# Malfoy/Brisk

Measured on AMD Instinct MI355X. Metric: distinct k-mers indexed/sec (k=63,m=21), higher is better.
Workload: dtype u64; 1 GPU; 1x MI355X: 50M synthetic 150 bp reads per GPU, k=63 m=21 b=14, uint8 counts, 15x coverage; reads_per_gpu=50000000, total_reads=50000000, part_bits=24, genome_len=500000000, parallelism=single GPU

## Files before the change

### brisk_amd/csrc/brisk_capi.hip

```cpp
#include "brisk_kernels.hip"

#include <algorithm>
#include <atomic>
#include <cerrno>
#include <chrono>
#include <cmath>
#include <cstdio>
#include <cstdlib>
#include <cstring>
#include <mutex>
#include <new>
#include <string>
#include <thread>
#include <vector>

#include <fcntl.h>
#include <sys/stat.h>
#include <unistd.h>

#include "../../include/brisk_hip.h"

#if !defined(__HIP_DEVICE_COMPILE__) && defined(__x86_64__)
#include <immintrin.h>
#define BRISK_HOST_AVX2 1
// ... 17 lines not shown
    size_t reserved = 0, mapped = 0, gran = 0;
    std::vector<hipMemGenericAllocationHandle_t> handles;
    std::vector<size_t> sizes;
};

constexpr size_t kPinBytes = 8192;
struct PendingEvent {
    int slot;
    hipEvent_t a, b;
};

struct Counters {
    struct Scan { unsigned long long n_rec; u32 overflow, pad; } scan;
    struct Touched { u32 n_touched, pad; unsigned long long need; } touched;
    struct Kmers { unsigned long long bound, n_long; } kmers;
    struct Work { u32 wc[2], n_left, n_clean; } work;
    struct Plan { u32 n_long, n_vr; } plan;
    u32 n_rerun, pad;
    unsigned long long kept;
    unsigned long long n_ovf;
    unsigned long long slice_sum;
    u32 upsert_done, pad2;
    struct Result { unsigned long long w[3]; } result;
    unsigned long long dbg_guard;
};
static_assert(sizeof(Counters::Scan) == sizeof(unsigned long long) + 2 * sizeof(u32) && sizeof(Counters::Touched) == 2 * sizeof(u32) + sizeof(unsigned long long), "ScanOut; k_touched, k_need");
static_assert(sizeof(Counters::Kmers) == 2 * sizeof(unsigned long long) && sizeof(Counters::Result) == 3 * sizeof(unsigned long long), "k_count_kmers: out[0..1]; k_checksum: out[0..2]");
static_assert(sizeof(Counters::Work) == 4 * sizeof(u32) && sizeof(Counters::Plan) == 2 * sizeof(u32), "32-bit counters throughout");
struct PinnedCounters : Counters {
    u32 n_huge;
    unsigned long long arena_used;
    unsigned long long n_rec_new;
    unsigned long long prof[3];
    unsigned long long answers;
};

}

struct brisk_hip_index {
    BriskParams P{};
    int device = 0;
    hipStream_t stream = nullptr;
    bool own_stream = false;
    std::string err;
    std::recursive_mutex call_mu;
    u64 n_parts = 0, n_buckets = 0;
    u64 max_batch_reads = 0;

    double* d_coef = nullptr;
    double* d_tabs = nullptr;
    ScanCfg scfg{};
    u64 dbg_guard_last = 0;
    bool fresh = true;
    u32 insert_waves = 4096;
    u32 scan_waves = 0;
    size_t scan_lds = 0;
    bool scan_v1 = false;
    bool entry_ids = false;
    u32 count_mode = 0;
    bool use_vmm = false;
    bool scan_hist_valid = false;
    u64 arena_limit = 0;
    VmBuf vm_keys, vm_counts, vm_ids;
    unsigned long long* d_id_counter = nullptr;
    DevBuf seq_buf;
    u64 arena_cap = 0;
// ... 407 lines not shown
    HIPCHK(h, zero_ctr(h, &h->d_ctr->touched));
    {
        ProfScope ps(h, S_TOUCHED);
        if ((rc = list_touched(h, &h->d_ctr->touched.n_touched))) return rc;
    }
    if (n_move) {
        if ((rc = ensure(h, h->parted, n_move * P.stride * 8))) return rc;
        ProfScope ps(h, S_SCATTER);
        const u64 n_slots = bl ? (u64)bl->ovf_region_cap * OVF_REGIONS : n_move;
        hipLaunchKernelGGL(k_scatter, dim3(nblocks(n_slots, 256)), dim3(256), 0, h->stream, P, bl ? (const u64*)bl->ovf : d_rec, n_move, h->d_cur32, (u64*)h->parted.p, 0,
                           (const u32*)nullptr, (u32*)nullptr, h->ix.err, bl ? bl->ovf_cnt : (const u32*)nullptr, bl ? bl->ovf_region_cap : 0u);
        if ((rc = launch_check(h, "k_scatter"))) return rc;
    }
    HIPCHK(h, fetch_ctr_sync(h, &h->d_ctr->touched.n_touched));
    const u32 n_touched = h->h_ctr->touched.n_touched;
    if (n_touched == 0) return BRISK_HIP_OK;
    static const long huge_env = getenv("BRISK_HUGE_AT") ? atol(getenv("BRISK_HUGE_AT")) : -1;
    const u32 huge_at = h->entry_ids ? 0u : huge_env >= 0 ? (u32)huge_env : 16384u;
    {
        ProfScope ps(h, S_TOUCHED);
        if ((rc = ensure(h, h->desc, (size_t)n_touched * sizeof(PartDesc)))) return rc;
        if (huge_at) {
            if ((rc = ensure(h, h->huge, (size_t)(HUGE_LIST_CAP + 1) * 4))) return rc;
            HIPCHK(h, hipMemsetAsync(h->huge.p, 0, 4, h->stream));
        }
        hipLaunchKernelGGL(k_need, dim3(std::min<u32>(nblocks(n_touched, 256), 2048)), dim3(256), 0, h->stream, h->d_hist, (bl && !n_move) ? (const u32*)nullptr : h->d_off,
                           h->d_touched, n_touched, h->ix.dir, (PartDesc*)h->desc.p, &h->d_ctr->touched.need, bl ? bl->bin_cap : 0u, huge_at, huge_at ? (u32*)h->huge.p : (u32*)nullptr,
                           (u32)HUGE_LIST_CAP);
        if (int lrc = launch_check(h, "k_need")) return lrc;
    }
// ... 16 lines not shown
        static const u32 wave_env = getenv("BRISK_INSERT_WAVES") ? (u32)atoi(getenv("BRISK_INSERT_WAVES")) : 0u;
        const bool sat = h->count_mode == BRISK_HIP_COUNTS_SATURATE;
        auto resident = [&](const void* fn, int cap_per_cu = 0) -> u32 {
            int per_cu = 0, cus = 0;
            if (hipOccupancyMaxActiveBlocksPerMultiprocessor(&per_cu, fn, 64, 0) != hipSuccess || per_cu <= 0) per_cu = 16;
            if (cap_per_cu && per_cu > cap_per_cu) per_cu = cap_per_cu;
            if (hipDeviceGetAttribute(&cus, hipDeviceAttributeMultiprocessorCount, h->device) != hipSuccess || cus <= 0) cus = 256;
            const u32 w = std::min<u32>((u32)per_cu * (u32)cus, h->insert_waves);
            static const bool dbg = getenv("BRISK_DEBUG_INSERT") != nullptr;
            if (dbg) fprintf(stderr, "[brisk_hip] k_insert: %d waves per CU x %d CUs resident, %u launched\n", per_cu, cus, wave_env ? std::min<u32>(w, wave_env) : w);
            return wave_env ? std::min<u32>(w, wave_env) : w;
        };
        static const bool generic_only = getenv("BRISK_INSERT_GENERIC") != nullptr;
        static const bool lean_off = getenv("BRISK_INSERT_LEAN") && !strcmp(getenv("BRISK_INSERT_LEAN"), "0");
        static const bool clean_off = getenv("BRISK_INSERT_CLEAN") && !strcmp(getenv("BRISK_INSERT_CLEAN"), "0");
        const bool lean = fresh && !generic_only && !lean_off && !h->entry_ids && !big && P.nw == 3 && P.kb == 49 && P.shift >= 1 && P.shift <= 4;
        if (lean) {
            if ((rc = ensure(h, h->left, (size_t)n_touched * 4))) return rc;
            static const bool dbg = getenv("BRISK_DEBUG_INSERT") != nullptr;
            if (dbg) {
                hipFuncAttributes fa{};
                int per_cu = 0;
                const void* fn = sat ? (const void*)k_insert_first<3, 49, 4, true> : (const void*)k_insert_first<3, 49, 4, false>;
                if (hipFuncGetAttributes(&fa, fn) == hipSuccess && hipOccupancyMaxActiveBlocksPerMultiprocessor(&per_cu, fn, 64, 0) == hipSuccess) {
                    fprintf(stderr, "[brisk_hip] k_insert_first: the occupancy query gives %d waves per CU, the kernel is built for at most %d\n", per_cu, 4 * WI_WAVES_PER_EU_FIRST_MAX);
                    per_cu = std::min(per_cu, 4 * WI_WAVES_PER_EU_FIRST_MAX);
                    fprintf(stderr, "[brisk_hip] k_insert_first: %d waves per CU, %d registers, %zu B of LDS, %zu B of scratch\n", per_cu, fa.numRegs, fa.sharedSizeBytes, fa.localSizeBytes);
                }
            }
        }
// ... 11 lines not shown
        else if (big) LAUNCH_INSERT_K(k_insert_big, NW, KB, SH, false)                                                                                              \
        else if (sat) LAUNCH_INSERT_K(k_insert, NW, KB, SH, true)                                                                                                   \
        else LAUNCH_INSERT_K(k_insert, NW, KB, SH, false)                                                                                                           \
    }
#define LAUNCH_INSERT_FAST(NW, KB, SH)                                                                                                                              \
    {                                                                                                                                                               \
        if (big) LAUNCH_INSERT(NW, KB, SH)                                                                                                                          \
        else if (sat) LAUNCH_INSERT_K(k_insert_fast, NW, KB, SH, true)                                                                                              \
        else LAUNCH_INSERT_K(k_insert_fast, NW, KB, SH, false)                                                                                                      \
    }
#define LAUNCH_INSERT_LEAN_K(SH, SAT)                                                                                                                               \
    {                                                                                                                                                               \
        u32* const wc = h->d_ctr->work.wc;                                                                                                                          \
        u32* const n_left = &h->d_ctr->work.n_left;                                                                                                                 \
        u32* const n_clean = clean_off ? nullptr : &h->d_ctr->work.n_clean;                                                                                         \
        body = "k_insert_first<3,49," #SH;                                                                                                                          \
        const dim3 grid(std::min<u32>(batches, resident((const void*)k_insert_first<3, 49, SH, SAT>, 4 * WI_WAVES_PER_EU_FIRST_MAX)));                                                            \
        hipLaunchKernelGGL((k_insert_first<3, 49, SH, SAT>), grid, dim3(64), 0, h->stream, P, src, (const PartDesc*)h->desc.p, n_touched, h->ix, wc,                \
                           (u32*)h->left.p, n_left, n_clean);                                                                                                       \
        if ((rc = launch_check(h, "k_insert_first"))) return rc;                                                                                                    \
        const dim3 grid2(std::min<u32>(batches, resident((const void*)k_insert_fast_listed<3, 49, SH, SAT>)));                                                     \
        hipLaunchKernelGGL((k_insert_fast_listed<3, 49, SH, SAT>), grid2, dim3(64), 0, h->stream, P, src, (const PartDesc*)h->desc.p, n_touched, h->ix, wc + 1,     \
                           (const u32*)h->left.p, (const u32*)n_left);                                                                                              \
    }
#define LAUNCH_INSERT_LEAN(SH)                                                                                                                                      \
    {                                                                                                                                                               \
        if (sat) LAUNCH_INSERT_LEAN_K(SH, true)                                                                                                                     \
        else LAUNCH_INSERT_LEAN_K(SH, false)                                                                                                                        \
    }
        if (lean && P.shift == 4) LAUNCH_INSERT_LEAN(4)
        else if (lean && P.shift == 3) LAUNCH_INSERT_LEAN(3)
        else if (lean && P.shift == 2) LAUNCH_INSERT_LEAN(2)
        else if (lean) LAUNCH_INSERT_LEAN(1)
        else if (!generic_only && P.nw == 3 && P.kb == 49 && P.shift == 4) LAUNCH_INSERT_FAST(3, 49, 4)
// ... 10 lines not shown
#undef LAUNCH_INSERT_FAST
#undef LAUNCH_INSERT
#undef LAUNCH_INSERT_K
        if ((rc = launch_check(h, big ? "k_insert_big" : "k_insert"))) return rc;
        if (h->trace) {
            std::string path = big ? "k_insert_big (in-place collapse for partitions of > 128 records)" : "k_insert", tail;
            if (lean) {
                HIPCHK(h, fetch_ctr_sync(h, &h->d_ctr->work));
                const u32 n_left = h->h_ctr->work.n_left;
                path = "k_insert_first (fresh index): " + std::to_string(n_touched - n_huge - n_left) + " partitions lean, " + std::to_string(n_left) + " left over to k_insert";
                tail = " (" + std::to_string(h->h_ctr->work.n_clean) + " table-free)";
            }
            fprintf(stderr, "[brisk_hip] path: insert of %llu records (%s layout, histogram %s) into %u partitions: %s, %u partitions to k_insert_huge%s\n", (unsigned long long)n_rec,
                    bl ? "binned" : "classic", have_hist ? "from the scan" : "counted here", n_touched, path.c_str(), n_huge, tail.c_str());
            fprintf(stderr, "[brisk_hip] body: %s,%s>%s\n", body, sat ? "sat" : "wrap", lean ? ", then k_insert_fast_listed" : "");
        }
        if (n_huge) {
            if (sat) hipLaunchKernelGGL(k_insert_huge<true>, dim3(std::min<u32>(n_huge, 256u)), dim3(HG_THREADS), 0, h->stream, P, src, (const PartDesc*)h->desc.p,
                                        (const u32*)h->huge.p + 1, (const u32*)h->huge.p, h->ix);
            else hipLaunchKernelGGL(k_insert_huge<false>, dim3(std::min<u32>(n_huge, 256u)), dim3(HG_THREADS), 0, h->stream, P, src, (const PartDesc*)h->desc.p,
                                    (const u32*)h->huge.p + 1, (const u32*)h->huge.p, h->ix);
            if ((rc = launch_check(h, "k_insert_huge"))) return rc;
        }
    }
    h->nb_skmers += n_rec;
    h->dir_snapshot_valid = false;
    return BRISK_HIP_OK;
}

int launch_scan(brisk_hip_index* h, const u32* d_packed, const u64* d_starts, u64 n_items, const ScanOut& out, bool query_mode, bool plain,
// ... 2889 lines not shown
#undef LAUNCH_DEBUG_KEYS
    if ((rc = launch_check(h, "k_debug_keys"))) return rc;
    HIPCHK(h, hipMemcpyAsync(keys, d_k, n * 8, hipMemcpyDeviceToHost, h->stream));
    HIPCHK(h, fetch_ctr_sync(h, &h->d_ctr->dbg_guard));
    h->dbg_guard_last = h->h_ctr->dbg_guard;
    return BRISK_HIP_OK;
}

BRISK_API int brisk_hip_debug_guard_count(brisk_hip_index* h, uint64_t* n_guard) {
    if (!h || !n_guard) return BRISK_HIP_EINVAL;
    std::lock_guard<std::recursive_mutex> call_lock(h->call_mu);
    *n_guard = h->dbg_guard_last;
    return BRISK_HIP_OK;
}

BRISK_API int brisk_hip_debug_host_pack(const char* bases, uint64_t n_bases, uint32_t* packed, int scalar) {
    if (n_bases && (!bases || !packed)) return BRISK_HIP_EINVAL;
    if (scalar) host_pack_scalar(bases, n_bases, packed);
    else host_pack(bases, n_bases, packed);
    return BRISK_HIP_OK;
}
#ifdef BRISK_PHASE_PROF
BRISK_API int brisk_hip_debug_scan_counts(uint64_t out[8], int reset) {
    if (hipMemcpyFromSymbol(out, HIP_SYMBOL(g_scan_cnt), 8 * 8) != hipSuccess) return BRISK_HIP_EHIP;
    if (reset) {
        uint64_t z[8] = {};
        if (hipMemcpyToSymbol(HIP_SYMBOL(g_scan_cnt), z, 8 * 8) != hipSuccess) return BRISK_HIP_EHIP;
    }
    return BRISK_HIP_OK;
}
// ... 41 lines not shown
```

### brisk_amd/csrc/brisk_insert.hip

```cpp
#ifndef ARENA_CHUNK
#define ARENA_CHUNK 16384u
#endif
#ifndef INSERT_SLOTS
#define INSERT_SLOTS 8192u
#endif
#ifndef WI_WAVES_PER_EU
#define WI_WAVES_PER_EU 4
#endif
#ifdef BRISK_PHASE_PROF
__device__ unsigned long long g_phase[16];
#define PHASE_DECL unsigned long long ph_acc[12] = {0, 0, 0, 0, 0, 0, 0, 0, 0, 0, 0, 0}; unsigned long long ph_last = __builtin_amdgcn_s_memtime(); u32 dbg_cnt[16] = {0, 0, 0, 0, 0, 0, 0, 0, 0, 0, 0, 0, 0, 0, 0, 0};
#define PHASE(i) { const unsigned long long t_ = __builtin_amdgcn_s_memtime(); ph_acc[i] += t_ - ph_last; ph_last = t_; }
__device__ unsigned long long g_cnt[16];
#define PHASE_FLUSH { PHASE(10) if (threadIdx.x == 0) { _Pragma("unroll") for (int q_ = 0; q_ < 12; q_++) atomicAdd(&g_phase[q_], ph_acc[q_]); \
                                                         _Pragma("unroll") for (int q_ = 0; q_ < 16; q_++) atomicAdd(&g_cnt[q_], (unsigned long long)dbg_cnt[q_]); } }
#define CNT(i, v) dbg_cnt[i] += (v);
#else
#define PHASE_DECL
#define PHASE(i)
#define PHASE_FLUSH
#define CNT(i, v)
#endif
struct IndexDev {
    u64* keys;
// ... 453 lines not shown
}

#ifndef FOLD_GROUPED
#define FOLD_GROUPED 1
#endif
#ifdef INSERT_ATTR_ONEROUND
#define FOLD_GROUPED_TRIPS 1u
#else
#define FOLD_GROUPED_TRIPS WI_FOLD_TRIPS
#endif
__device__ __forceinline__ u32 fold_slot(u32 ck) { return (ck * 0x9E3779B1u) >> 26; }
__device__ __forceinline__ u32 lane_fetch(u32 v, u32 a4) { return (u32)__builtin_amdgcn_ds_bpermute((int)a4, (int)v); }
__device__ __forceinline__ u64 lane_fetch64(u64 v, u32 a4) { return ((u64)lane_fetch((u32)(v >> 32), a4) << 32) | lane_fetch((u32)v, a4); }
template <u32 NW>
__device__ __forceinline__ bool fold_records_grouped(const FoldFrame& f, u32 nrec, u32 lane, u32* s_slot, u32* lead, u32* off, bool* folded_out, u32* trips, u32 ck, bool unsure,
                                                     bool* clean) {
    static_assert(WI_FOLD_TRIPS < (1u << 18), "[round | n | 63 - lane] in 32 bits: n < 256, so sv < 1 << 14");
    if (__any(unsure)) return false;
    u32 sv = lane < nrec ? f.s : 0;
    bool folded = false;
    u32 dirty = 0, heads = 0;
    *lead = lane;
    *off = 0;
    u32* my_slot = s_slot + fold_slot(ck);
    s_slot[lane] = 0;
    wave_sync();
    for (u32 t = 1; t <= FOLD_GROUPED_TRIPS; t++) {
        if (!__any(sv != 0) || heads > WI_FOLD_TRIPS) break;
        *trips += 1;
        const u32 mine = (t << 14) | sv;
        if (sv != 0) atomicMax(my_slot, mine);
// ... 11 lines not shown
        in = in && same;
        if (in) {
            sv = 0;
            if (lane != a) {
                folded = true;
                *lead = a;
                *off = i0 - i0a;
            }
        }
        const u32 meets = ((i0 - ea) & (i0a - e)) >> 31;
        dirty |= (ck_a == ck && sv != 0) ? meets : 0u;
    }
#ifndef INSERT_ATTR_ONEROUND
    if (heads > WI_FOLD_TRIPS || __any(sv != 0)) return false;
#endif
    *clean = !__any(dirty != 0);
    *folded_out = folded;
    return true;
}

template <u32 MAXI, u32 NW, u32 KB, u32 SHIFT, bool SAT, bool LISTED = false>
__device__ __forceinline__ void insert_body(const BriskParams& PP, const RecSrc& src, const PartDesc* __restrict__ desc, u32 n_touched_all, const IndexDev& ix,
                                            u32* __restrict__ work_counter, const u32* __restrict__ list = nullptr, const u32* __restrict__ n_list = nullptr) {
    const u32 n_touched = LISTED ? min(*n_list, n_touched_all) : n_touched_all;
    u64* const rec = src.rec;
    BriskParams P = PP;
    if (NW) {
        P.nw = NW;
        P.stride = NW + 1;
        P.kb = KB;
        P.shift = SHIFT;
// ... 427 lines not shown
#ifndef WI_WAVES_PER_EU_FIRST_MAX
#define WI_WAVES_PER_EU_FIRST_MAX 6
#endif
template <u32 NIL, u32 NW>
struct LeanLds {
    static constexpr u32 MAXI = 64 * NIL, TABLE = 512;
    static_assert((TABLE & (TABLE - 1)) == 0 && TABLE >= 2 * MAXI && TABLE <= 4 * MAXI, "probe table: a power of two, at most half full");
    static constexpr u32 REC_BYTES = (WI_MAX_REC * RecGeom<NW>::RS + 4) * 4;
    static constexpr u32 OFF_REC = 16 * MAXI;
    static constexpr u32 REGION = REC_BYTES > 4 * TABLE ? REC_BYTES : 4 * TABLE;
    static constexpr u32 OFF_IREC = OFF_REC + REGION, OFF_IMULT = OFF_IREC + MAXI, BYTES = OFF_IMULT + MAXI;
};
__device__ __forceinline__ unsigned long long first_lane64(unsigned long long v) {
    return ((unsigned long long)(u32)__builtin_amdgcn_readfirstlane((int)(v >> 32)) << 32) | (u32)__builtin_amdgcn_readfirstlane((int)v);
}
template <u32 NIL, u32 NW, u32 KB, u32 SHIFT, bool SAT>
__device__ __forceinline__ void insert_first_body(const BriskParams& P, const RecSrc& src, const PartDesc* __restrict__ desc, u32 n_touched, const IndexDev& ix,
                                                  u32* __restrict__ work_counter, u32* __restrict__ left_list, u32* __restrict__ n_left, u32* __restrict__ n_clean) {
    using L = LeanLds<NIL, NW>;
    constexpr u32 MAXI = L::MAXI, TABLE = L::TABLE, RS = RecGeom<NW>::RS, INFO = RecGeom<NW>::INFO, KBITS = 2 * KB + 6;
    constexpr u32 KW = KBITS + SHIFT <= 64 ? 1u : 2u;
    constexpr u32 CORE_K = 63, CORE_M = 21, CORE_B = 14, CW = CORE_K - CORE_M;
    static_assert(KB == CORE_K - CORE_B, "fold_core: the core of k63 m21 b14");
    static_assert(NIL == 2 || NIL == 3, "instance slots per lane");
    static_assert(NW >= 3 && SHIFT < 5, "the folding k63 geometries: at most 16 buckets per partition");
    static_assert(L::BYTES <= 13 * 512, "LDS per wave: 24 waves must fit a CU's 160 KiB");
    static_assert(4 * MAXI <= 16 * MAXI, "the multiplicity steps lie over the keys");
    static_assert(MAXI + (MAXI >> 2) + 8 <= ARENA_CHUNK / 8, "grow_cap(MAXI) is a small request: the host's arena reserve covers the tail a refill strands");
    __shared__ __attribute__((aligned(16))) unsigned char s_mem[L::BYTES];
    u64* s_key = (u64*)s_mem;
    u32* s_idiff = (u32*)s_mem;
    u32* s_rw = (u32*)(s_mem + L::OFF_REC);
    u32* s_tab = (u32*)(s_mem + L::OFF_REC);
    uint8_t* s_irec = s_mem + L::OFF_IREC;
    uint8_t* s_imult = s_mem + L::OFF_IMULT;

    const u32 lane = threadIdx.x;
    PHASE_DECL
    unsigned long long acur = first_lane64(ix.slot_cur[blockIdx.x]), aend = first_lane64(ix.slot_end[blockIdx.x]), garbage = 0;
    const u32 frame_end = P.suff_reduc + P.w + 1;
    const u32 core_from = (n_clean != nullptr && P.w == CW) ? P.suff_reduc : 0x100u;

    for (;;) {
        u32 t0 = 0;
        if (lane == 0) t0 = atomicAdd(work_counter, WI_BATCH);
        t0 = (u32)__builtin_amdgcn_readfirstlane((int)t0);
        if (t0 >= n_touched) break;
        const u32 t_end = min(t0 + WI_BATCH, n_touched);
        unsigned long long left_mask = 0;
        unsigned long long clean_mask = 0;
        PartDesc d = desc[t0];
        RecRegs rr = load_part_recs(P, src, d.part, d.r_begin, d.r_begin, min(d.n_rec, (u32)WI_MAX_REC), lane);

        for (u32 t = t0; t < t_end; t++) {
            const u32 tn = t + 1;
            PartDesc dn{};
            if (tn < t_end) dn = desc[tn];
            asm volatile("" ::"v"(rr.w0), "v"(rr.w1), "v"(rr.w2), "v"(rr.w3), "v"(rr.w4));
            do {
                if (ix.huge_at && d.n_inst > ix.huge_at) break;
                CNT(0, 1)
                if (d.n_exist | d.cap | (u32)(d.n_rec > WI_MAX_REC)) {
                    left_mask |= 1ull << (t - t0);
                    break;
                }
                PHASE(0)
                const u32 part = d.part, nrec = d.n_rec;
                const u64 my_hdr = NW == 3 ? rr.w3 : rr.w4;
                const u32 raw_n = lane < nrec ? hdr_n(my_hdr) : 0;
                const u32 my_mult = (my_hdr & HDR_HAS_MULT) ? (u32)(my_hdr >> 48) & 0xffu : 1u;
                const u32 info_hi = (raw_n << 10) | (hdr_idx0(my_hdr) << 18) | ((hdr_bucket(my_hdr) & ((1u << SHIFT) - 1)) << 26);
                const FoldFrame ff = fold_frame<NW, KB>(rr, my_hdr, raw_n, lane < nrec, frame_end, lane);
                wave_sync();
                if (lane < nrec) store_rec_words<NW>(s_rw + lane * RS, rr, 0);
                u32 lead = lane, lead_off = 0, dbg_trips = 0;
                const bool unsure = lane < nrec && (ff.s == 0 || hdr_idx0(my_hdr) < core_from);
                bool clean = false;
                const u32 ck = ((hdr_bucket(my_hdr) & ((1u << SHIFT) - 1)) << (2 * (KB - CW))) | fold_core<KB, CW>(ff.u);
                bool dup = false;
                if (!FOLD_GROUPED || !fold_records_grouped<NW>(ff, nrec, lane, (u32*)s_mem, &lead, &lead_off, &dup, &dbg_trips, ck, unsure, &clean))
                    dup = fold_records<NW, true>(ff, nrec, lane, &lead, &lead_off, &dbg_trips, ck, unsure, &clean);
#ifdef INSERT_ATTR_NOTABLE
                clean = true;
#endif
                const u32 my_n = (lane < nrec && !dup) ? raw_n : 0;
                const u32 x = wave_incl_scan(my_n, lane);
                const u32 ninst = (u32)__builtin_amdgcn_readlane((int)x, 63);
                if (ninst > MAXI) {
                    left_mask |= 1ull << (t - t0);
                    break;
                }
                PHASE(1)
                CNT(1, 1)
                const u32 m_first = (u32)__shfl(x - my_n, lead, 64) + lead_off;
                u32 tsize = 128;
                while (tsize < 4 * ninst && tsize < TABLE) tsize <<= 1;
                {
                    if (NIL == 2) ((uint16_t*)s_irec)[lane] = 0;
                    else {
#pragma unroll
                        for (u32 q = 0; q < NIL; q++) s_irec[q * 64 + lane] = 0;
                    }
// ... 40 lines not shown
                        }
                    }
                    if (lane < nrec) s_rw[lane * RS + INFO] = (x - my_n) | info_hi;
                }
                wave_sync();
                PHASE(2)
                CNT(3, (ninst + 63) / 64)
                CNT(4, ninst)
                CNT(5, nrec)
                CNT(11, dbg_trips)
                u32 dbg_r = 0;
                LaneInst<NIL> li;
                li.won = 0;
                u32 n_new = 0, new_rank[NIL], new_word[NIL];
                if (clean) {
                    clean_mask |= 1ull << (t - t0);
                    u32 ln = lane;
                    asm volatile("" : "+v"(ln));
                    if (ninst <= 64) expand_words_distinct<1, NW, KB, SHIFT, NIL>(ln, ninst, s_rw, s_irec, li);
                    else if (NIL == 2 || ninst <= 128) expand_words_distinct<2, NW, KB, SHIFT, NIL>(ln, ninst, s_rw, s_irec, li);
                    else expand_words_distinct<NIL, NW, KB, SHIFT, NIL>(ln, ninst, s_rw, s_irec, li);
                    n_new = ninst;
#pragma unroll
                    for (u32 it = 0; it < NIL; it++) {
                        const u32 i = it * 64 + ln;
                        new_rank[it] = i;
                        new_word[it] = (u32)s_imult[i < ninst ? i : 0] << WI_CNT_SHIFT;
                    }
                    PHASE(3)
                } else {
                    if (ninst <= 64) expand_and_dedupe_words<1, NW, KB, SHIFT, NIL, true, SAT>(lane, ninst, tsize, s_rw, s_irec, s_imult, nullptr, s_key, s_tab, &dbg_r, li);
// ... 9 lines not shown
                        if (it * 64 < ninst) {
                            const bool made = (li.won >> it) & 1;
                            if (made) new_word[it] = s_tab[li.hh[it]];
                            const unsigned long long bal = __ballot(made);
                            new_rank[it] = n_new + (u32)__popcll(bal & lanes_below(lane));
                            n_new += (u32)__popcll(bal);
                        }
                    }
                }
                wave_sync();
#ifndef INSERT_NO_EARLY_WAIT
                __builtin_amdgcn_s_waitcnt(0x0F70);
#endif
                PHASE(6)
                CNT(7, n_new)
                unsigned long long off = d.off;
                u32 cap = 0;
                if (n_new) {
                    const unsigned long long want = grow_cap(n_new);
                    if (acur + want > aend) {
                        garbage += aend - acur;
                        unsigned long long got = 0;
                        if (lane == 0) got = atomicAdd(ix.cursor, (unsigned long long)ARENA_CHUNK);
                        acur = first_lane64(got);
                        aend = acur + ARENA_CHUNK;
                    }
                    if (acur + want > ix.arena_cap) {
                        if (lane == 0) atomicOr(ix.err, 2u);
                        n_new = 0;
                    } else {
                        off = acur;
                        acur += want;
                        cap = (u32)want;
                    }
                }
                PHASE(7)
                u32 bm0 = 0;
#pragma unroll
                for (u32 it = 0; it < NIL; it++) {
                    if (it * 64 < ninst && ((li.won >> it) & 1) && n_new) {
                        const unsigned long long at = off + new_rank[it];
                        store_key<KW>(ix, at, li.klo[it], li.khi[it]);
                        ix.counts[at] = (uint8_t)count8<SAT>(new_word[it] >> WI_CNT_SHIFT);
                        const u32 bl = SHIFT ? ((u32)shr128(mk128(li.klo[it], li.khi[it]), KBITS).lo & ((1u << SHIFT) - 1)) : 0;
                        bm0 |= 1u << bl;
                    }
                }
                PHASE(8)
                bm0 = wave_or_all(bm0);
                if (lane == 0) {
                    ix.dir[part] = DirEnt{off, n_new, cap};
                    const u64 first = ((u64)part << SHIFT) >> P.ext_bits;
                    const u32 bits = bm0 << (first & 31);
                    if (bits && (!ix.bits_check || (ix.bucket_bits[first >> 5] & bits) != bits)) atomicOr(&ix.bucket_bits[first >> 5], bits);
                }
            } while (0);
            d = dn;
            if (tn < t_end) rr = load_part_recs(P, src, d.part, d.r_begin, d.r_begin, min(d.n_rec, (u32)WI_MAX_REC), lane);
            PHASE(9)
        }
        if (left_mask) {
            const u32 n = (u32)__popcll(left_mask);
            u32 at = 0;
            if (lane == 0) at = atomicAdd(n_left, n);
            at = (u32)__builtin_amdgcn_readfirstlane((int)at);
            u32 ln = lane;
            asm volatile("" : "+v"(ln));
            if ((left_mask >> ln) & 1) left_list[at + (u32)__popcll(left_mask & lanes_below(ln))] = t0 + ln;
        }
        if (clean_mask && n_clean && lane == 0) atomicAdd(n_clean, (u32)__popcll(clean_mask));
    }
    PHASE_FLUSH
    if (lane == 0) {
        ix.slot_cur[blockIdx.x] = acur;
        ix.slot_end[blockIdx.x] = aend;
        if (garbage) atomicAdd(&ix.stats[3], garbage);
    }
}
template <u32 NW, u32 KB, u32 SHIFT, bool SAT = false, u32 NIL = NI_LEAN>
__global__ void __launch_bounds__(64) __attribute__((amdgpu_waves_per_eu(WI_WAVES_PER_EU_FIRST, WI_WAVES_PER_EU_FIRST_MAX))) k_insert_first(BriskParams P, RecSrc src, const PartDesc* __restrict__ desc,
                                                                                                          u32 n_touched, IndexDev ix, u32* __restrict__ work_counter,
                                                                                                          u32* __restrict__ left_list, u32* __restrict__ n_left, u32* __restrict__ n_clean) {
    insert_first_body<NIL, NW, KB, SHIFT, SAT>(P, src, desc, n_touched, ix, work_counter, left_list, n_left, n_clean);
}

__global__ void __launch_bounds__(256) k_bucket_bits(BriskParams P, IndexDev ix, u32 n_parts) {
    const u32 kbits = 2 * P.kb + 6;
    for (u32 part = blockIdx.x; part < n_parts; part += gridDim.x) {
        const u32 cnt = ix.dir[part].cnt;
        const unsigned long long off = ix.dir[part].off;
        for (u32 e = threadIdx.x; e < cnt; e += blockDim.x) {
            const u128x key = load_key(ix, off + e);
            const u32 bucket = (part << P.shift) | ((u32)shr128(key, kbits).lo & ((1u << P.shift) - 1));
            const u32 bit = 1u << (bucket & 31);
            if (!(ix.bucket_bits[bucket >> 5] & bit)) atomicOr(&ix.bucket_bits[bucket >> 5], bit);
        }
    }
}
// ... 229 lines not shown
```

### brisk_amd/hipapi.py

```python
from __future__ import annotations

import atexit
import ctypes as C
import math
import os
import subprocess
import sys
import weakref
from typing import Optional, Sequence, Tuple

import numpy as np

HERE = os.path.dirname(os.path.abspath(__file__))
ROOT = os.path.dirname(HERE)
_LIB_NAME = os.environ.get("BRISK_HIP_LIB", "libbrisk_hip.so")

STATUS = {0: "OK", 1: "EINVAL", 2: "EUNSUPPORTED", 3: "EHIP", 4: "ENOMEM", 5: "ECAPACITY", 6: "ENODEVICE", 7: "EIO", 8: "EFORMAT"}
ECAPACITY = 5


class BriskHipError(RuntimeError):
    def __init__(self, code: int, msg: str = ""):
        self.code = code
        super().__init__(f"brisk_hip: {STATUS.get(code, code)} {msg}".strip())
# ... 72 lines not shown

class _JointWindow(C.Structure):
    _fields_ = [(n, C.c_uint32) for n in ("min_self", "max_self", "min_other", "max_other", "keep_absent", "reserved")]


JOINT_ABSENT = 256
JOINT_STATES = 257

_u64p = np.ctypeslib.ndpointer(dtype=np.uint64, flags="C_CONTIGUOUS")
_u8p = np.ctypeslib.ndpointer(dtype=np.uint8, flags="C_CONTIGUOUS")

SYMBOLS = [
    "brisk_hip_abi_version", "brisk_hip_create", "brisk_hip_destroy", "brisk_hip_clear", "brisk_hip_last_error", "brisk_hip_sync",
    "brisk_hip_get_layout", "brisk_hip_insert_reads", "brisk_hip_insert_packed", "brisk_hip_get_reads", "brisk_hip_lookup",
    "brisk_hip_enumerate", "brisk_hip_stats", "brisk_hip_memory_info", "brisk_hip_insert_slack", "brisk_hip_reallocate", "brisk_hip_checksum", "brisk_hip_scan_packed", "brisk_hip_scan_bound", "brisk_hip_route_records",
    "brisk_hip_get_packed", "brisk_hip_get_kmers", "brisk_hip_get_kmers_packed", "brisk_hip_insert_records", "brisk_hip_set_owner_cuts", "brisk_hip_export_hist", "brisk_hip_export_hist_add", "brisk_hip_insert_records_hist", "brisk_hip_scan_query", "brisk_hip_route_tagged", "brisk_hip_query_records", "brisk_hip_pack_ascii", "brisk_hip_synth_reads", "brisk_hip_debug_order_keys", "brisk_hip_debug_guard_count", "brisk_hip_scan_sequence", "brisk_hip_upsert_kmers", "brisk_hip_find_kmers",
    "brisk_hip_enumerate_ids", "brisk_hip_count_spectrum", "brisk_hip_enumerate_range", "brisk_hip_prune",
    "brisk_hip_read_profile_reads", "brisk_hip_read_profile_packed",
    "brisk_hip_scan_kmers", "brisk_hip_record_kmers", "brisk_hip_answer_records", "brisk_hip_place_answers", "brisk_hip_profile_slots",
    "brisk_hip_select_intervals", "brisk_hip_extract_packed", "brisk_hip_trim_packed", "brisk_hip_trim_reads", "brisk_hip_unpack_ascii",
    "brisk_hip_intake_ascii", "brisk_hip_intake_reads", "brisk_hip_insert_raw_reads",
    "brisk_hip_fragment_intervals", "brisk_hip_pair_intervals", "brisk_hip_compose_intervals", "brisk_hip_extract_pairs_packed",
    "brisk_hip_trim_pairs_packed", "brisk_hip_trim_pairs_reads", "brisk_hip_clean_pairs_ascii", "brisk_hip_clean_pairs_reads",
    "brisk_hip_merge", "brisk_hip_intersect", "brisk_hip_subtract", "brisk_hip_compare", "brisk_hip_joint_spectrum", "brisk_hip_filter_joint", "brisk_hip_snapshot_info_read", "brisk_hip_save", "brisk_hip_load",
    "brisk_hip_profile_enable",
    "brisk_hip_profile_read", "brisk_hip_profile_reset",
]

_lib = None


# ... 923 lines not shown
        dts = (np.uint64, np.uint64, np.uint8, np.uint32)
        return tuple(np.concatenate(a) if a else np.zeros(0, dt) for a, dt in zip(out, dts))

    def debug_order_keys(self, mmers, exact: bool = False) -> np.ndarray:
        x = np.ascontiguousarray(mmers, np.uint64)
        out = np.zeros(max(len(x), 1), np.uint64)
        self._chk(self.L.brisk_hip_debug_order_keys(self.h, x, len(x), 1 if exact else 0, out))
        return out[: len(x)]

    def debug_guard_count(self) -> int:
        n = C.c_uint64(0)
        self.L.brisk_hip_debug_guard_count.argtypes = [C.c_void_p, C.POINTER(C.c_uint64)]
        self._chk(self.L.brisk_hip_debug_guard_count(self.h, C.byref(n)))
        return int(n.value)

    def profile_enable(self, on: bool = True):
        self._chk(self.L.brisk_hip_profile_enable(self.h, 1 if on else 0))

    def profile_reset(self):
        self._chk(self.L.brisk_hip_profile_reset(self.h))

    def profile_read(self) -> dict:
        n = C.c_uint32()
        names = (C.c_char_p * 16)()
        launches = (C.c_uint64 * 16)()
        ms = (C.c_double * 16)()
        self._chk(self.L.brisk_hip_profile_read(self.h, C.byref(n), names, launches, ms))
        return {names[i].decode(): {"launches": launches[i], "ms": ms[i]} for i in range(n.value)}
```

### include/brisk_hip.h

```cpp
#ifndef BRISK_HIP_H
#define BRISK_HIP_H

#include <stddef.h>
#include <stdint.h>

#ifdef __cplusplus
extern "C" {
#endif

#define BRISK_HIP_ABI_VERSION 4

enum {
    BRISK_HIP_OK = 0,
    BRISK_HIP_EINVAL = 1,
    BRISK_HIP_EUNSUPPORTED = 2,
    BRISK_HIP_EHIP = 3,
    BRISK_HIP_ENOMEM = 4,
    BRISK_HIP_ECAPACITY = 5,
    BRISK_HIP_ENODEVICE = 6,
    BRISK_HIP_EIO = 7,
    BRISK_HIP_EFORMAT = 8
};

typedef struct brisk_hip_index brisk_hip_index;
// ... 251 lines not shown
int brisk_hip_upsert_kmers(brisk_hip_index *h, const uint64_t *kmer_lo, const uint64_t *kmer_hi, const uint8_t *minimizer_idx,
                           uint64_t n, uint32_t *ids, uint8_t *newly);
int brisk_hip_find_kmers(brisk_hip_index *h, const uint64_t *kmer_lo, const uint64_t *kmer_hi, const uint8_t *minimizer_idx,
                         uint64_t n, uint32_t *ids);
int brisk_hip_enumerate_ids(brisk_hip_index *h, uint64_t *cursor, uint64_t *out_lo, uint64_t *out_hi,
                            uint8_t *out_minimizer_idx, uint32_t *out_ids, uint64_t cap, uint64_t *n_out);

int brisk_hip_pack_ascii(brisk_hip_index *h, const char *d_bases, uint64_t n_bases, uint32_t *d_packed);
int brisk_hip_unpack_ascii(brisk_hip_index *h, const uint32_t *d_packed, uint64_t first_nt, uint64_t n_nts, char *d_bases);
int brisk_hip_synth_reads(brisk_hip_index *h, uint64_t genome_len, uint64_t first_read, uint64_t n_reads,
                          uint32_t read_len, uint64_t seed_g, uint64_t seed_r,
                          uint32_t *d_packed, uint64_t *d_starts);

int brisk_hip_debug_order_keys(brisk_hip_index *h, const uint64_t *mmers, uint64_t n, int exact, uint64_t *keys);
int brisk_hip_debug_guard_count(brisk_hip_index *h, uint64_t *n_guard);

#define BRISK_HIP_PROFILE_SLOTS 16
int brisk_hip_profile_enable(brisk_hip_index *h, int on);
int brisk_hip_profile_read(brisk_hip_index *h, uint32_t *n_slots, const char **names, uint64_t *launches, double *ms);
int brisk_hip_profile_reset(brisk_hip_index *h);

#ifdef __cplusplus
}
#endif
#endif
```

Before: 33.91 billion k-mers/s.

## Pair adjacent small fresh partitions into one wave pass in k_insert_first

In the lean first-insert kernel, two consecutive fresh partitions whose combined record count fits in one wave are now loaded and folded together, with a partition bit added to the fold key so their records stay apart. If both fold cleanly and fit the instance limit, both partitions are processed and written in a single iteration, and the loop advances by two. Otherwise the code falls back to the first partition alone. The aim is to reduce idle lanes and per-partition overhead when many partitions hold only a few records, at the cost of extra branching, register pressure and refold work when a pair fails. Debug accessors for touched partitions and directory entries are also added.

```diff
diff --git a/brisk_amd/csrc/brisk_capi.hip b/brisk_amd/csrc/brisk_capi.hip
--- a/brisk_amd/csrc/brisk_capi.hip
+++ b/brisk_amd/csrc/brisk_capi.hip
@@ -55,7 +55,7 @@
     struct Scan { unsigned long long n_rec; u32 overflow, pad; } scan;
     struct Touched { u32 n_touched, pad; unsigned long long need; } touched;
     struct Kmers { unsigned long long bound, n_long; } kmers;
-    struct Work { u32 wc[2], n_left, n_clean; } work;
+    struct Work { u32 wc[2], n_left, n_clean, n_pair, pad; } work;
     struct Plan { u32 n_long, n_vr; } plan;
     u32 n_rerun, pad;
     unsigned long long kept;
@@ -67,7 +67,7 @@
 };
 static_assert(sizeof(Counters::Scan) == sizeof(unsigned long long) + 2 * sizeof(u32) && sizeof(Counters::Touched) == 2 * sizeof(u32) + sizeof(unsigned long long), "ScanOut; k_touched, k_need");
 static_assert(sizeof(Counters::Kmers) == 2 * sizeof(unsigned long long) && sizeof(Counters::Result) == 3 * sizeof(unsigned long long), "k_count_kmers: out[0..1]; k_checksum: out[0..2]");
-static_assert(sizeof(Counters::Work) == 4 * sizeof(u32) && sizeof(Counters::Plan) == 2 * sizeof(u32), "32-bit counters throughout");
+static_assert(sizeof(Counters::Work) == 6 * sizeof(u32) && sizeof(Counters::Plan) == 2 * sizeof(u32), "32-bit counters throughout");
 struct PinnedCounters : Counters {
     u32 n_huge;
     unsigned long long arena_used;
@@ -91,6 +91,7 @@
     double* d_coef = nullptr;
     double* d_tabs = nullptr;
     ScanCfg scfg{};
+    u32 dbg_touched_last = 0;
     u64 dbg_guard_last = 0;
     bool fresh = true;
     u32 insert_waves = 4096;
@@ -528,6 +529,7 @@
     }
     HIPCHK(h, fetch_ctr_sync(h, &h->d_ctr->touched.n_touched));
     const u32 n_touched = h->h_ctr->touched.n_touched;
+    h->dbg_touched_last = n_touched;
     if (n_touched == 0) return BRISK_HIP_OK;
     static const long huge_env = getenv("BRISK_HUGE_AT") ? atol(getenv("BRISK_HUGE_AT")) : -1;
     const u32 huge_at = h->entry_ids ? 0u : huge_env >= 0 ? (u32)huge_env : 16384u;
@@ -574,6 +576,7 @@
         static const bool generic_only = getenv("BRISK_INSERT_GENERIC") != nullptr;
         static const bool lean_off = getenv("BRISK_INSERT_LEAN") && !strcmp(getenv("BRISK_INSERT_LEAN"), "0");
         static const bool clean_off = getenv("BRISK_INSERT_CLEAN") && !strcmp(getenv("BRISK_INSERT_CLEAN"), "0");
+        static const bool pair_off = getenv("BRISK_INSERT_PAIR") && !strcmp(getenv("BRISK_INSERT_PAIR"), "0");
         const bool lean = fresh && !generic_only && !lean_off && !h->entry_ids && !big && P.nw == 3 && P.kb == 49 && P.shift >= 1 && P.shift <= 4;
         if (lean) {
             if ((rc = ensure(h, h->left, (size_t)n_touched * 4))) return rc;
@@ -615,10 +618,11 @@
         u32* const wc = h->d_ctr->work.wc;                                                                                                                          \
         u32* const n_left = &h->d_ctr->work.n_left;                                                                                                                 \
         u32* const n_clean = clean_off ? nullptr : &h->d_ctr->work.n_clean;                                                                                         \
+        u32* const n_pair = (clean_off || pair_off) ? nullptr : &h->d_ctr->work.n_pair;                                                                             \
         body = "k_insert_first<3,49," #SH;                                                                                                                          \
         const dim3 grid(std::min<u32>(batches, resident((const void*)k_insert_first<3, 49, SH, SAT>, 4 * WI_WAVES_PER_EU_FIRST_MAX)));                                                            \
         hipLaunchKernelGGL((k_insert_first<3, 49, SH, SAT>), grid, dim3(64), 0, h->stream, P, src, (const PartDesc*)h->desc.p, n_touched, h->ix, wc,                \
-                           (u32*)h->left.p, n_left, n_clean);                                                                                                       \
+                           (u32*)h->left.p, n_left, n_clean, n_pair);                                                                                               \
         if ((rc = launch_check(h, "k_insert_first"))) return rc;                                                                                                    \
         const dim3 grid2(std::min<u32>(batches, resident((const void*)k_insert_fast_listed<3, 49, SH, SAT>)));                                                     \
         hipLaunchKernelGGL((k_insert_fast_listed<3, 49, SH, SAT>), grid2, dim3(64), 0, h->stream, P, src, (const PartDesc*)h->desc.p, n_touched, h->ix, wc + 1,     \
@@ -659,6 +663,14 @@
             fprintf(stderr, "[brisk_hip] path: insert of %llu records (%s layout, histogram %s) into %u partitions: %s, %u partitions to k_insert_huge%s\n", (unsigned long long)n_rec,
                     bl ? "binned" : "classic", have_hist ? "from the scan" : "counted here", n_touched, path.c_str(), n_huge, tail.c_str());
             fprintf(stderr, "[brisk_hip] body: %s,%s>%s\n", body, sat ? "sat" : "wrap", lean ? ", then k_insert_fast_listed" : "");
+        }
+        if (lean) {
+            static const bool dbg = getenv("BRISK_DEBUG_INSERT") != nullptr;
+            if (dbg) {
+                HIPCHK(h, fetch_ctr_sync(h, &h->d_ctr->work));
+                fprintf(stderr, "[brisk_hip] k_insert_first: %u of %u partitions taken in pairs, %u table-free, %u left over\n", h->h_ctr->work.n_pair, n_touched,
+                        h->h_ctr->work.n_clean, h->h_ctr->work.n_left);
+            }
         }
         if (n_huge) {
             if (sat) hipLaunchKernelGGL(k_insert_huge<true>, dim3(std::min<u32>(n_huge, 256u)), dim3(HG_THREADS), 0, h->stream, P, src, (const PartDesc*)h->desc.p,
@@ -3578,6 +3590,33 @@
     return BRISK_HIP_OK;
 }
 
+BRISK_API int brisk_hip_debug_touched(brisk_hip_index* h, uint32_t* parts, uint64_t cap, uint64_t* n) {
+    if (!h || !n || (cap && !parts)) return BRISK_HIP_EINVAL;
+    HIPCHK(h, hipSetDevice(h->device));
+    std::lock_guard<std::recursive_mutex> call_lock(h->call_mu);
+    *n = h->dbg_touched_last;
+    const u64 take = std::min<u64>(cap, h->dbg_touched_last);
+    if (take) HIPCHK(h, hipMemcpyAsync(parts, h->d_touched, take * 4, hipMemcpyDeviceToHost, h->stream));
+    HIPCHK(h, hipStreamSynchronize(h->stream));
+    return BRISK_HIP_OK;
+}
+
+BRISK_API int brisk_hip_debug_directory(brisk_hip_index* h, const uint32_t* parts, uint64_t n, uint32_t* cnt, uint32_t* cap) {
+    if (!h || (n && (!parts || !cnt || !cap))) return BRISK_HIP_EINVAL;
+    HIPCHK(h, hipSetDevice(h->device));
+    std::lock_guard<std::recursive_mutex> call_lock(h->call_mu);
+    for (u64 i = 0; i < n; i++)
+        if (parts[i] >= h->n_parts) return BRISK_HIP_EINVAL;
+    std::vector<DirEnt> dir(h->n_parts);
+    HIPCHK(h, hipMemcpyAsync(dir.data(), h->ix.dir, h->n_parts * sizeof(DirEnt), hipMemcpyDeviceToHost, h->stream));
+    HIPCHK(h, hipStreamSynchronize(h->stream));
+    for (u64 i = 0; i < n; i++) {
+        cnt[i] = dir[parts[i]].cnt;
+        cap[i] = dir[parts[i]].cap;
+    }
+    return BRISK_HIP_OK;
+}
+
 BRISK_API int brisk_hip_debug_host_pack(const char* bases, uint64_t n_bases, uint32_t* packed, int scalar) {
     if (n_bases && (!bases || !packed)) return BRISK_HIP_EINVAL;
     if (scalar) host_pack_scalar(bases, n_bases, packed);
diff --git a/brisk_amd/csrc/brisk_insert.hip b/brisk_amd/csrc/brisk_insert.hip
--- a/brisk_amd/csrc/brisk_insert.hip
+++ b/brisk_amd/csrc/brisk_insert.hip
@@ -491,7 +491,7 @@
 __device__ __forceinline__ u64 lane_fetch64(u64 v, u32 a4) { return ((u64)lane_fetch((u32)(v >> 32), a4) << 32) | lane_fetch((u32)v, a4); }
 template <u32 NW>
 __device__ __forceinline__ bool fold_records_grouped(const FoldFrame& f, u32 nrec, u32 lane, u32* s_slot, u32* lead, u32* off, bool* folded_out, u32* trips, u32 ck, bool unsure,
-                                                     bool* clean) {
+                                                     bool* clean, unsigned long long* dirty_lanes = nullptr) {
     static_assert(WI_FOLD_TRIPS < (1u << 18), "[round | n | 63 - lane] in 32 bits: n < 256, so sv < 1 << 14");
     if (__any(unsure)) return false;
     u32 sv = lane < nrec ? f.s : 0;
@@ -533,7 +533,9 @@
 #ifndef INSERT_ATTR_ONEROUND
     if (heads > WI_FOLD_TRIPS || __any(sv != 0)) return false;
 #endif
-    *clean = !__any(dirty != 0);
+    const unsigned long long dl = __ballot(dirty != 0);
+    if (dirty_lanes) *dirty_lanes = dl;
+    *clean = dl == 0;
     *folded_out = folded;
     return true;
 }
@@ -991,9 +993,33 @@
 __device__ __forceinline__ unsigned long long first_lane64(unsigned long long v) {
     return ((unsigned long long)(u32)__builtin_amdgcn_readfirstlane((int)(v >> 32)) << 32) | (u32)__builtin_amdgcn_readfirstlane((int)v);
 }
+#ifndef INSERT_PAIR
+#define INSERT_PAIR 1
+#endif
+#define PAIR_B_BIT 18u
+__device__ __forceinline__ RecRegs load_pair_recs(const BriskParams& P, const RecSrc& src, u32 part_a, u32 begin_a, u32 nA, u32 part_b, u32 begin_b, u32 nB, u32 lane) {
+    RecRegs r{0, 0, 0, 0, 0};
+    const u32 in_bin = src.bin_cap ? src.bin_cap : ~0u;
+    const u64 bytes = (u64)P.stride * 8, rec0 = (u64)(uintptr_t)src.rec, ovf0 = (u64)(uintptr_t)src.ovf;
+    const u64 bin_a = rec0 + (src.bin_cap ? (u64)part_a * src.bin_cap : (u64)begin_a) * bytes, ovf_a = ovf0 + ((u64)begin_a - src.bin_cap) * bytes;
+    const u64 bin_b = rec0 + (src.bin_cap ? (u64)part_b * src.bin_cap : (u64)begin_b) * bytes, ovf_b = ovf0 + ((u64)begin_b - src.bin_cap) * bytes;
+    if (lane < nA + nB) {
+        const bool is_b = lane >= nA;
+        const u32 i = is_b ? lane - nA : lane;
+        const u64 base = i < in_bin ? (is_b ? bin_b : bin_a) : (is_b ? ovf_b : ovf_a);
+        const u64* c = (const u64*)(uintptr_t)(base + i * bytes);
+        r.w0 = c[0];
+        r.w1 = c[1];
+        if (P.stride > 2) r.w2 = c[2];
+        if (P.stride > 3) r.w3 = c[3];
+        if (P.stride > 4) r.w4 = c[4];
+    }
+    return r;
+}
 template <u32 NIL, u32 NW, u32 KB, u32 SHIFT, bool SAT>
 __device__ __forceinline__ void insert_first_body(const BriskParams& P, const RecSrc& src, const PartDesc* __restrict__ desc, u32 n_touched, const IndexDev& ix,
-                                                  u32* __restrict__ work_counter, u32* __restrict__ left_list, u32* __restrict__ n_left, u32* __restrict__ n_clean) {
+                                                  u32* __restrict__ work_counter, u32* __restrict__ left_list, u32* __restrict__ n_left, u32* __restrict__ n_clean,
+                                                  u32* __restrict__ n_pair) {
     using L = LeanLds<NIL, NW>;
     constexpr u32 MAXI = L::MAXI, TABLE = L::TABLE, RS = RecGeom<NW>::RS, INFO = RecGeom<NW>::INFO, KBITS = 2 * KB + 6;
     constexpr u32 KW = KBITS + SHIFT <= 64 ? 1u : 2u;
@@ -1017,6 +1043,20 @@
     unsigned long long acur = first_lane64(ix.slot_cur[blockIdx.x]), aend = first_lane64(ix.slot_end[blockIdx.x]), garbage = 0;
     const u32 frame_end = P.suff_reduc + P.w + 1;
     const u32 core_from = (n_clean != nullptr && P.w == CW) ? P.suff_reduc : 0x100u;
+    const bool pair_on = INSERT_PAIR && n_pair != nullptr && core_from != 0x100u;
+    auto request = [&](const PartDesc& a, u32 ta, u32 t_end, RecRegs& rr) -> u32 {
+        u32 nB = 0, part_b = 0, begin_b = 0;
+        if (pair_on && ta + 1 < t_end && !(a.n_exist | a.cap) && a.n_rec - 1u < (u32)WI_MAX_REC - 1u && !(ix.huge_at && a.n_inst > ix.huge_at)) {
+            const PartDesc b = desc[ta + 1];
+            if (!(b.n_exist | b.cap) && b.n_rec != 0 && a.n_rec + b.n_rec <= (u32)WI_MAX_REC && !(ix.huge_at && b.n_inst > ix.huge_at)) {
+                nB = b.n_rec;
+                part_b = b.part;
+                begin_b = b.r_begin;
+            }
+        }
+        rr = load_pair_recs(P, src, a.part, a.r_begin, min(a.n_rec, (u32)WI_MAX_REC), part_b, begin_b, nB, lane);
+        return nB;
+    };
 
     for (;;) {
         u32 t0 = 0;
@@ -1026,11 +1066,15 @@
         const u32 t_end = min(t0 + WI_BATCH, n_touched);
         unsigned long long left_mask = 0;
         unsigned long long clean_mask = 0;
+        u32 pairs = 0;
         PartDesc d = desc[t0];
-        RecRegs rr = load_part_recs(P, src, d.part, d.r_begin, d.r_begin, min(d.n_rec, (u32)WI_MAX_REC), lane);
-
-        for (u32 t = t0; t < t_end; t++) {
-            const u32 tn = t + 1;
+        RecRegs rr;
+        u32 nB = INSERT_PAIR ? request(d, t0, t_end, rr) : 0u;
+        if (!INSERT_PAIR) rr = load_part_recs(P, src, d.part, d.r_begin, d.r_begin, min(d.n_rec, (u32)WI_MAX_REC), lane);
+
+        for (u32 t = t0, step = 1; t < t_end; t += step) {
+            u32 tn = t + 1;
+            step = 1;
             PartDesc dn{};
             if (tn < t_end) dn = desc[tn];
             asm volatile("" ::"v"(rr.w0), "v"(rr.w1), "v"(rr.w2), "v"(rr.w3), "v"(rr.w4));
@@ -1042,7 +1086,8 @@
                     break;
                 }
                 PHASE(0)
-                const u32 part = d.part, nrec = d.n_rec;
+                const u32 part = d.part, nA = d.n_rec;
+                u32 nrec = nA + nB;
                 const u64 my_hdr = NW == 3 ? rr.w3 : rr.w4;
                 const u32 raw_n = lane < nrec ? hdr_n(my_hdr) : 0;
                 const u32 my_mult = (my_hdr & HDR_HAS_MULT) ? (u32)(my_hdr >> 48) & 0xffu : 1u;
@@ -1051,18 +1096,45 @@
                 wave_sync();
                 if (lane < nrec) store_rec_words<NW>(s_rw + lane * RS, rr, 0);
                 u32 lead = lane, lead_off = 0, dbg_trips = 0;
-                const bool unsure = lane < nrec && (ff.s == 0 || hdr_idx0(my_hdr) < core_from);
+                const bool unsure_any = ff.s == 0 || hdr_idx0(my_hdr) < core_from;
                 bool clean = false;
-                const u32 ck = ((hdr_bucket(my_hdr) & ((1u << SHIFT) - 1)) << (2 * (KB - CW))) | fold_core<KB, CW>(ff.u);
+                const u32 ck = ((hdr_bucket(my_hdr) & ((1u << SHIFT) - 1)) << (2 * (KB - CW))) | fold_core<KB, CW>(ff.u) |
+                               (INSERT_PAIR && lane >= nA ? 1u << PAIR_B_BIT : 0u);
+                static_assert(SHIFT + 2 * (KB - CW) <= PAIR_B_BIT, "ck: the partition bit lies above the routing id's low bits and the core");
                 bool dup = false;
-                if (!FOLD_GROUPED || !fold_records_grouped<NW>(ff, nrec, lane, (u32*)s_mem, &lead, &lead_off, &dup, &dbg_trips, ck, unsure, &clean))
+                unsigned long long dirty_lanes = 0;
+                for (;;) {
+                    const bool unsure = lane < nrec && unsure_any;
+                    if (FOLD_GROUPED && fold_records_grouped<NW>(ff, nrec, lane, (u32*)s_mem, &lead, &lead_off, &dup, &dbg_trips, ck, unsure, &clean, &dirty_lanes)) break;
+                    if (INSERT_PAIR && nB) {
+                        nB = 0;
+                        nrec = nA;
+                        continue;
+                    }
                     dup = fold_records<NW, true>(ff, nrec, lane, &lead, &lead_off, &dbg_trips, ck, unsure, &clean);
+                    break;
+                }
 #ifdef INSERT_ATTR_NOTABLE
                 clean = true;
 #endif
-                const u32 my_n = (lane < nrec && !dup) ? raw_n : 0;
+                u32 my_n = (lane < nrec && !dup) ? raw_n : 0;
                 const u32 x = wave_incl_scan(my_n, lane);
-                const u32 ninst = (u32)__builtin_amdgcn_readlane((int)x, 63);
+                u32 ninst = (u32)__builtin_amdgcn_readlane((int)x, 63);
+                u32 ninstA = ninst;
+                if (INSERT_PAIR && nB) {
+                    ninstA = (u32)__builtin_amdgcn_readlane((int)x, (int)(nA - 1));
+                    const bool clean_a = (dirty_lanes & ((1ull << nA) - 1)) == 0;
+                    if (clean && ninst <= MAXI) {
+                        step = 2;
+                        pairs += 2;
+                    } else {
+                        nB = 0;
+                        nrec = nA;
+                        clean = clean_a;
+                        if (lane >= nA) my_n = 0;
+                        ninst = ninstA;
+                    }
+                }
                 if (ninst > MAXI) {
                     left_mask |= 1ull << (t - t0);
                     break;
@@ -1133,7 +1205,7 @@
                 li.won = 0;
                 u32 n_new = 0, new_rank[NIL], new_word[NIL];
                 if (clean) {
-                    clean_mask |= 1ull << (t - t0);
+                    clean_mask |= (INSERT_PAIR && nB ? 3ull : 1ull) << (t - t0);
                     u32 ln = lane;
                     asm volatile("" : "+v"(ln));
                     if (ninst <= 64) expand_words_distinct<1, NW, KB, SHIFT, NIL>(ln, ninst, s_rw, s_irec, li);
@@ -1173,26 +1245,61 @@
 #endif
                 PHASE(6)
                 CNT(7, n_new)
+                auto take_slice = [&](u32& n, unsigned long long& off, u32& cap) {
+                    cap = 0;
+                    if (n) {
+                        const unsigned long long want = grow_cap(n);
+                        if (acur + want > aend) {
+                            garbage += aend - acur;
+                            unsigned long long got = 0;
+                            if (lane == 0) got = atomicAdd(ix.cursor, (unsigned long long)ARENA_CHUNK);
+                            acur = first_lane64(got);
+                            aend = acur + ARENA_CHUNK;
+                        }
+                        if (acur + want > ix.arena_cap) {
+                            if (lane == 0) atomicOr(ix.err, 2u);
+                            n = 0;
+                        } else {
+                            off = acur;
+                            acur += want;
+                            cap = (u32)want;
+                        }
+                    }
+                };
+                if (INSERT_PAIR && nB) {
+                    unsigned long long off = d.off, off_b = dn.off;
+                    u32 cap = 0, cap_b = 0, n_new_b = n_new - ninstA;
+                    n_new = ninstA;
+                    take_slice(n_new, off, cap);
+                    take_slice(n_new_b, off_b, cap_b);
+                    u32 ln = lane, bm0 = 0;
+                    asm volatile("" : "+v"(ln));
+#pragma unroll
+                    for (u32 it = 0; it < NIL; it++) {
+                        const u32 i = it * 64 + ln;
+                        const bool in_b = i >= ninstA;
+                        if (i < ninst && (in_b ? n_new_b : n_new)) {
+                            const unsigned long long at = (in_b ? off_b - ninstA : off) + i;
+                            store_key<KW>(ix, at, li.klo[it], li.khi[it]);
+                            ix.counts[at] = (uint8_t)count8<SAT>(new_word[it] >> WI_CNT_SHIFT);
+                            const u32 bl = (u32)shr128(mk128(li.klo[it], li.khi[it]), KBITS).lo & ((1u << SHIFT) - 1);
+                            bm0 |= 1u << (bl + (in_b ? 16u : 0u));
+                        }
+                    }
+                    bm0 = wave_or_all(bm0);
+                    if (ln == 0) {
+                        ix.dir[part] = DirEnt{off, n_new, cap};
+                        ix.dir[dn.part] = DirEnt{off_b, n_new_b, cap_b};
+                        const u64 first = ((u64)part << SHIFT) >> P.ext_bits, first_b = ((u64)dn.part << SHIFT) >> P.ext_bits;
+                        const u32 bits = (bm0 & 0xffffu) << (first & 31), bits_b = (bm0 >> 16) << (first_b & 31);
+                        if (bits && (!ix.bits_check || (ix.bucket_bits[first >> 5] & bits) != bits)) atomicOr(&ix.bucket_bits[first >> 5], bits);
+                        if (bits_b && (!ix.bits_check || (ix.bucket_bits[first_b >> 5] & bits_b) != bits_b)) atomicOr(&ix.bucket_bits[first_b >> 5], bits_b);
+                    }
+                    break;
+                }
                 unsigned long long off = d.off;
                 u32 cap = 0;
-                if (n_new) {
-                    const unsigned long long want = grow_cap(n_new);
-                    if (acur + want > aend) {
-                        garbage += aend - acur;
-                        unsigned long long got = 0;
-                        if (lane == 0) got = atomicAdd(ix.cursor, (unsigned long long)ARENA_CHUNK);
-                        acur = first_lane64(got);
-                        aend = acur + ARENA_CHUNK;
-                    }
-                    if (acur + want > ix.arena_cap) {
-                        if (lane == 0) atomicOr(ix.err, 2u);
-                        n_new = 0;
-                    } else {
-                        off = acur;
-                        acur += want;
-                        cap = (u32)want;
-                    }
-                }
+                take_slice(n_new, off, cap);
                 PHASE(7)
                 u32 bm0 = 0;
 #pragma unroll
@@ -1214,10 +1321,19 @@
                     if (bits && (!ix.bits_check || (ix.bucket_bits[first >> 5] & bits) != bits)) atomicOr(&ix.bucket_bits[first >> 5], bits);
                 }
             } while (0);
+            if (INSERT_PAIR && step == 2) {
+                tn = t + 2;
+                dn = PartDesc{};
+                if (tn < t_end) dn = desc[tn];
+            }
             d = dn;
-            if (tn < t_end) rr = load_part_recs(P, src, d.part, d.r_begin, d.r_begin, min(d.n_rec, (u32)WI_MAX_REC), lane);
+            if (INSERT_PAIR) {
+                nB = 0;
+                if (tn < t_end) nB = request(d, tn, t_end, rr);
+            } else if (tn < t_end) rr = load_part_recs(P, src, d.part, d.r_begin, d.r_begin, min(d.n_rec, (u32)WI_MAX_REC), lane);
             PHASE(9)
         }
+        if (INSERT_PAIR && pairs && lane == 0) atomicAdd(n_pair, pairs);
         if (left_mask) {
             const u32 n = (u32)__popcll(left_mask);
             u32 at = 0;
@@ -1239,8 +1355,9 @@
 template <u32 NW, u32 KB, u32 SHIFT, bool SAT = false, u32 NIL = NI_LEAN>
 __global__ void __launch_bounds__(64) __attribute__((amdgpu_waves_per_eu(WI_WAVES_PER_EU_FIRST, WI_WAVES_PER_EU_FIRST_MAX))) k_insert_first(BriskParams P, RecSrc src, const PartDesc* __restrict__ desc,
                                                                                                           u32 n_touched, IndexDev ix, u32* __restrict__ work_counter,
-                                                                                                          u32* __restrict__ left_list, u32* __restrict__ n_left, u32* __restrict__ n_clean) {
-    insert_first_body<NIL, NW, KB, SHIFT, SAT>(P, src, desc, n_touched, ix, work_counter, left_list, n_left, n_clean);
+                                                                                                          u32* __restrict__ left_list, u32* __restrict__ n_left, u32* __restrict__ n_clean,
+                                                                                                          u32* __restrict__ n_pair) {
+    insert_first_body<NIL, NW, KB, SHIFT, SAT>(P, src, desc, n_touched, ix, work_counter, left_list, n_left, n_clean, n_pair);
 }
 
 __global__ void __launch_bounds__(256) k_bucket_bits(BriskParams P, IndexDev ix, u32 n_parts) {
diff --git a/brisk_amd/hipapi.py b/brisk_amd/hipapi.py
--- a/brisk_amd/hipapi.py
+++ b/brisk_amd/hipapi.py
@@ -110,7 +110,7 @@
     "brisk_hip_abi_version", "brisk_hip_create", "brisk_hip_destroy", "brisk_hip_clear", "brisk_hip_last_error", "brisk_hip_sync",
     "brisk_hip_get_layout", "brisk_hip_insert_reads", "brisk_hip_insert_packed", "brisk_hip_get_reads", "brisk_hip_lookup",
     "brisk_hip_enumerate", "brisk_hip_stats", "brisk_hip_memory_info", "brisk_hip_insert_slack", "brisk_hip_reallocate", "brisk_hip_checksum", "brisk_hip_scan_packed", "brisk_hip_scan_bound", "brisk_hip_route_records",
-    "brisk_hip_get_packed", "brisk_hip_get_kmers", "brisk_hip_get_kmers_packed", "brisk_hip_insert_records", "brisk_hip_set_owner_cuts", "brisk_hip_export_hist", "brisk_hip_export_hist_add", "brisk_hip_insert_records_hist", "brisk_hip_scan_query", "brisk_hip_route_tagged", "brisk_hip_query_records", "brisk_hip_pack_ascii", "brisk_hip_synth_reads", "brisk_hip_debug_order_keys", "brisk_hip_debug_guard_count", "brisk_hip_scan_sequence", "brisk_hip_upsert_kmers", "brisk_hip_find_kmers",
+    "brisk_hip_get_packed", "brisk_hip_get_kmers", "brisk_hip_get_kmers_packed", "brisk_hip_insert_records", "brisk_hip_set_owner_cuts", "brisk_hip_export_hist", "brisk_hip_export_hist_add", "brisk_hip_insert_records_hist", "brisk_hip_scan_query", "brisk_hip_route_tagged", "brisk_hip_query_records", "brisk_hip_pack_ascii", "brisk_hip_synth_reads", "brisk_hip_debug_order_keys", "brisk_hip_debug_guard_count", "brisk_hip_debug_touched", "brisk_hip_debug_directory", "brisk_hip_scan_sequence", "brisk_hip_upsert_kmers", "brisk_hip_find_kmers",
     "brisk_hip_enumerate_ids", "brisk_hip_count_spectrum", "brisk_hip_enumerate_range", "brisk_hip_prune",
     "brisk_hip_read_profile_reads", "brisk_hip_read_profile_packed",
     "brisk_hip_scan_kmers", "brisk_hip_record_kmers", "brisk_hip_answer_records", "brisk_hip_place_answers", "brisk_hip_profile_slots",
@@ -1064,6 +1064,23 @@
         self._chk(self.L.brisk_hip_debug_guard_count(self.h, C.byref(n)))
         return int(n.value)
 
+    def debug_touched(self) -> np.ndarray:
+        f = self.L.brisk_hip_debug_touched
+        f.argtypes = [C.c_void_p, C.c_void_p, C.c_uint64, C.POINTER(C.c_uint64)]
+        n = C.c_uint64(0)
+        self._chk(f(self.h, None, 0, C.byref(n)))
+        out = np.zeros(max(int(n.value), 1), np.uint32)
+        self._chk(f(self.h, out.ctypes.data, len(out), C.byref(n)))
+        return out[: int(n.value)]
+
+    def debug_directory(self, parts):
+        f = self.L.brisk_hip_debug_directory
+        f.argtypes = [C.c_void_p, C.c_void_p, C.c_uint64, C.c_void_p, C.c_void_p]
+        p = np.ascontiguousarray(parts, np.uint32)
+        cnt, cap = np.zeros(max(len(p), 1), np.uint32), np.zeros(max(len(p), 1), np.uint32)
+        self._chk(f(self.h, p.ctypes.data, len(p), cnt.ctypes.data, cap.ctypes.data))
+        return cnt[: len(p)], cap[: len(p)]
+
     def profile_enable(self, on: bool = True):
         self._chk(self.L.brisk_hip_profile_enable(self.h, 1 if on else 0))
 
diff --git a/include/brisk_hip.h b/include/brisk_hip.h
--- a/include/brisk_hip.h
+++ b/include/brisk_hip.h
@@ -289,6 +289,8 @@
 
 int brisk_hip_debug_order_keys(brisk_hip_index *h, const uint64_t *mmers, uint64_t n, int exact, uint64_t *keys);
 int brisk_hip_debug_guard_count(brisk_hip_index *h, uint64_t *n_guard);
+int brisk_hip_debug_touched(brisk_hip_index *h, uint32_t *parts, uint64_t cap, uint64_t *n);
+int brisk_hip_debug_directory(brisk_hip_index *h, const uint32_t *parts, uint64_t n, uint32_t *cnt, uint32_t *cap);
 
 #define BRISK_HIP_PROFILE_SLOTS 16
 int brisk_hip_profile_enable(brisk_hip_index *h, int on);
```

After: 34.65 billion k-mers/s, median of 6. 1.02x the previous value.
